# calmiLovesAI/ComputerVision.pytorch

Hardware: AMD Instinct MI355X
Metric: images/sec 640x640 YOLOv8-n train step (higher is better)
Workload: dtype f16; 1 GPU; YOLOv8-n train step (fwd + v8 loss + bwd + Adam), batch 32/GPU, 640x640, nc=80, random init; global_batch=32, parallelism=dp1, launch=eager, exchange=none (1 rank), gpu_max_hw_queues=4

## Files before the change

__graft_entry__.py:

```python
import os
import subprocess
import sys

ROOT = os.path.dirname(os.path.abspath(__file__))
CSRC = os.path.join(ROOT, "computervision.pytorch_amd", "csrc")
LIBDIR = os.path.join(ROOT, "computervision.pytorch_amd", "lib")
LIB = os.path.join(LIBDIR, "libcvx_engine.so")
SOURCES = ["conv_igemm.hip", "conv_igemm_dma.hip", "conv_halo.hip", "conv_tile.hip", "conv_tile_k1.hip", "conv_tile_k2.hip", "conv_gemm.hip", "conv_stem7.hip", "conv_pw.hip", "conv_wgrad.hip", "conv_wgrad_gemm.hip", "conv_wgrad_halo.hip", "conv_wgrad_stream.hip", "conv_wgrad_k3.hip", "bn_act.hip", "stem.hip", "unit_ops.hip", "misc_ops.hip", "loss_v8.hip", "loss_seg.hip", "loss_seg_opts.hip", "loss_centernet.hip", "loss_multibox.hip", "loss_yolov7.hip", "preprocess.hip", "augment.hip", "seg_pipeline.hip", "det_eval.hip", "coco_eval.hip", "nms.hip", "centernet_decode.hip", "render.hip", "tiles.hip", "seg_tiles.hip", "seg_tta.hip", "det_tta.hip", "track.hip", "optim.hip", "comm.hip", "engine.hip"]


def _stale(out, deps):
    if not os.path.exists(out):
        return True
    t = os.path.getmtime(out)
    return any(os.path.getmtime(d) > t for d in deps)


def build(force: bool = False) -> None:
    os.makedirs(LIBDIR, exist_ok=True)
    objdir = os.path.join(ROOT, "build", "obj")
    os.makedirs(objdir, exist_ok=True)
    headers = [os.path.join(CSRC, f) for f in os.listdir(CSRC) if f.endswith(".h")] + [os.path.join(ROOT, "include", "cvx_engine.h")]
    hipcc = os.environ.get("HIPCC", "/opt/rocm/bin/hipcc")
    objs, procs = [], []
    for src in SOURCES:
        s = os.path.join(CSRC, src)
        o = os.path.join(objdir, src.replace(".hip", ".o"))
        objs.append(o)
        if force or _stale(o, [s] + headers):
            cmd = [hipcc, "--offload-arch=gfx950", "-O3", "-std=c++17", "-fPIC", "-c", s, "-o", o]
            procs.append((src, subprocess.Popen(cmd, stdout=subprocess.PIPE, stderr=subprocess.STDOUT, text=True)))
    for src, p in procs:
        out, _ = p.communicate()
        if p.returncode != 0:
            raise RuntimeError(f"hipcc failed on {src}:\n{out}")
    if force or procs or _stale(LIB, objs):
        cmd = [hipcc, "--offload-arch=gfx950", "-shared", "-fPIC", "-o", LIB] + objs
        r = subprocess.run(cmd, stdout=subprocess.PIPE, stderr=subprocess.STDOUT, text=True)
        if r.returncode != 0:
            raise RuntimeError("link failed:\n" + r.stdout)
    if ROOT not in sys.path:
# ... 46 lines not shown
```

computervision.pytorch_amd/_lib.py:

```python
from __future__ import annotations

import ctypes as C
import os

import numpy as np

_HERE = os.path.dirname(os.path.abspath(__file__))
LIB_PATH = os.environ.get("CVX_LIB") or os.path.join(_HERE, "lib", "libcvx_engine.so")
ABI_VERSION = 4
SEG_OPTS_KEY_OFFSET = 4096


class CvxError(RuntimeError):
    pass


class BufDesc(C.Structure):
    _fields_ = [("h", C.c_int32), ("w", C.c_int32), ("c", C.c_int32), ("kind", C.c_int32)]


class View(C.Structure):
    _fields_ = [("buf", C.c_int32), ("coff", C.c_int32), ("c", C.c_int32), ("pix_off", C.c_int32)]


# ... 20 lines not shown

_P, _I32, _I64, _F, _U64 = C.c_void_p, C.c_int32, C.c_int64, C.c_float, C.c_uint64

EXPERIMENTAL_PROTOTYPES = {
    "cvx_chain_pair_unit": (_I32, [_P, _I32, _I32, _I32, _I32, _P, _P, _P, _P, _P, _P, _I32, _P, _I32, _I32, _I32, C.POINTER(_F), _P]),
    "cvx_chain_conv_unit": (_I32, [_P, _I32, _I32, _I32, _I32, _P, _I32, _I32, _I32, _I32, _P, _P, _I32, _P, _I32, _I32, _I32, C.POINTER(_F), _P]),
    "cvx_chain_detect_unit": (_I32, [_P, _I32, _I32, _I32, _I32, _I32, _I32, _I32, _P, _P, _P, _P, _P, _P, _P, _P, _P, _P, _P, _I32, _I32, _I32,
                                     _I32, _I32, C.POINTER(_F), _P]),
    "cvx_wgrad_time_unit": (_I32, [_P, _P, _I32, _I32, _I32, _I32, _I32, _I32, _I32, _I32, _I32, _I32, _P, _I64, C.POINTER(_F), C.POINTER(_I32), _P]),
}

PROTOTYPES = {
    "cvx_last_error": (C.c_char_p, []),
    "cvx_abi_version": (_I32, []),
    "cvx_engine_create": (_I32, [C.POINTER(_P), C.POINTER(BufDesc), _I32, C.POINTER(OpDesc), _I32, _I32, _I32, _I32, _P]),
    "cvx_engine_destroy": (_I32, [_P]),
    "cvx_engine_bind": (_I32, [_P, _P, _P, _I64, _P, _I64]),
    "cvx_engine_set_bn": (_I32, [_P, _F, _F]),
    "cvx_engine_forward": (_I32, [_P, _P, _I32, _I32, _P]),
    "cvx_engine_backward": (_I32, [_P, _P, _F]),
    "cvx_engine_backward_begin": (_I32, [_P, _P, _F]),
    "cvx_engine_backward_range": (_I32, [_P, _I32, _I32]),
    "cvx_engine_grads_ready": (_I32, [_P, _I32, _I32, _P]),
    "cvx_engine_backward_end": (_I32, [_P]),
    "cvx_engine_workspace_bytes": (_I64, [_P]),
    "cvx_engine_plan_generation": (_I64, [_P]),
    "cvx_engine_debug_copy": (_I32, [_P, _I32, _I32, _P, _I64]),
    "cvx_engine_profile": (_I32, [_P, _I32]),
    "cvx_engine_profile_read": (_I32, [_P, _I32, C.POINTER(C.c_double), C.POINTER(C.c_double), C.POINTER(C.c_double),
                                       C.POINTER(_I64)]),
    "cvx_debug_clock_buffer": (_I32, [_P]),
    "cvx_debug_conv_tile_plan": (_I32, [_I32, _I32, _I32, _I32, _I32, _P]),
    "cvx_debug_conv_dma_plan": (_I32, [_I64, _I32, _I32, _I32, _P]),
    "cvx_engine_profile_dump": (_I32, [_P, C.c_char_p]),
    "cvx_pred_level_to_nchw": (_I32, [_P, _I32, _I32, _I32, _I32, _I32, _I32, _P, _P]),
    "cvx_nchw_grad_to_dpred": (_I32, [_P, _I32, _I32, _I32, _I32, _I32, _I32, _F, _P, _P]),
    "cvx_loss_v8_workspace_bytes": (_I64, [_I32, _I32, _I32, _I32]),
    "cvx_loss_v8": (_I32, [_P, _I32, _I32, _I32, _P, _I32, _I32, C.POINTER(_I32), C.POINTER(_F), _I32, _F, _F, _F, _F, _P, _P, _P,
                           _I64, _P]),
    "cvx_loss_v8_strided": (_I32, [_P, _I32, _I32, _I32, _I32, _P, _I32, _I32, C.POINTER(_I32), C.POINTER(_F), _I32, _F, _F, _F, _F, _P, _P, _P,
                                   _I64, _P]),
    "cvx_loss_v8_assignment": (_I32, [_P, _I32, _I32, _I32, _P, _P, _P]),
    "cvx_pack_targets": (_I32, [_P, _P, _P, _I32, _P, _P]),
    "cvx_decode_strided": (_I32, [_P, _I32, _I32, _I32, _I32, C.POINTER(_I32), C.POINTER(_F), _I32, _P, _P]),
    "cvx_adam_step": (_I32, [_P, _P, _P, _P, _I64, _F, _F, _F, _F, _I32, _P, _I32, _P]),
    "cvx_check_finite": (_I32, [_P, _I64, _P, _P]),
    "cvx_adam_step_dev": (_I32, [_P, _P, _P, _P, _I64, _F, _F, _F, _P, _P, _I32, _F, _P]),
    "cvx_ema_update": (_I32, [_P, _P, _I64, _F, _F, _P]),
    "cvx_adam_ema_step_dev": (_I32, [_P, _P, _P, _P, _I64, _F, _F, _F, _P, _P, _I32, _F, _P, _F, _F, _P]),
    "cvx_optim_step": (_I32, [_I32, _P, _P, _P, _P, _I64, _P, _P, _I32, _P, _F, _F, _F, _P, _I32, _F, _P, _P, _F, _F, _P]),
    "cvx_grad_norm_workspace": (_I64, [_I64]),
    "cvx_grad_norm": (_I32, [_P, _I64, _P, _P, _I32, _F, _F, _P, _P, _P, _I64, _P]),
    "cvx_engine_set_stream": (_I32, [_P, _P]),
    "cvx_engine_exchange_stream": (_P, [_P]),
    "cvx_decode": (_I32, [_P, _I32, _I32, _I32, C.POINTER(_I32), C.POINTER(_F), _I32, _P, _P]),
    "cvx_yolo7_decode": (_I32, [_P, _I32, _I32, _I32, _P, _P, _I32, _I32, _I32, _P, _P, _P]),
    "cvx_ssd_decode": (_I32, [_P, _P, _P, _I32, _I32, _I32, _F, _F, _P, _P, _P]),
    "cvx_ssd_decode_max": (_I32, [_P, _P, _P, _I32, _I32, _I32, _F, _F, _P, _P, _P, _P]),
    "cvx_pred_cols_to_nchw": (_I32, [_P, _I32, _I32, _I32, _I32, _I32, _I32, _I32, _P, _I64, _I64, _P]),
    "cvx_nms_workspace_bytes": (_I64, [_I32, _I32]),
    "cvx_nms": (_I32, [_P, _I32, _I32, _I32, _F, _F, _I32, _P, _P, _P, _P, _I64, _P]),
    "cvx_nms_variant": (_I32, [_P, _I32, _I32, _I32, _F, _F, _I32, _I32, _P, _P, _P, _P, _I64, _P]),
    "cvx_centernet_decode_workspace_bytes": (_I64, [_I32, _I32, _I32, _I32]),
    "cvx_centernet_decode": (_I32, [_P, _I32, _I32, _I32, _I32, _I32, _I32, _I32, _I32, _F, _F, _I32, _P, _P, _P, _P, _P, _P, _P, _I64, _P]),
    "cvx_conv2d_nhwc": (_I32, [_P, _I32, _I32, _I32, _I32, _P, _I32, _I32, _I32, _I32, _I32, _I32, _P, _P, _P, _P]),
    "cvx_conv2d_dgrad_nhwc": (_I32, [_P, _I32, _I32, _I32, _I32, _P, _I32, _I32, _I32, _I32, _I32, _P, _P]),
    "cvx_conv2d_wgrad_workspace_bytes": (_I64, [_I32, _I32, _I32, _I32, _I32, _I32]),
    "cvx_conv2d_wgrad_nhwc": (_I32, [_P, _P, _I32, _I32, _I32, _I32, _I32, _I32, _I32, _I32, _I32, _P, _P, _I64, _P]),
    "cvx_bn_silu_train_nhwc": (_I32, [_P, _I32, _I32, _I32, _P, _P, _F, _F, _P, _P, _P, _P, _P, _P, _P, _P]),
    "cvx_bn_silu_bwd_nhwc": (_I32, [_P, _P, _I32, _I32, _I32, _P, _P, _P, _F, _P, _P, _P, _P, _I32, _P]),
    "cvx_letterbox_geometry": (_I32, [_I32, _I32, _I32, _I32, _P, _P, _P, _P, _P]),
    "cvx_letterbox_u8_to_nchw": (_I32, [_P, _I32, _I32, _I32, _I32, _P, _I32, _I32, _P]),
    "cvx_letterbox_batch_u8_to_nchw": (_I32, [_P, _I32, _I32, _I32, _P, _I32, _I32, _P]),
    "cvx_det_to_image": (_I32, [_P, _P, _I32, _I32, _I32, _P, _P, _P, _P, _P]),
    "cvx_draw_detections": (_I32, [_P, _I32, _I32, _I32, _P, _P, _I32, _P, _I32, _I32, _I32, _P]),
    "cvx_seg_overlay": (_I32, [_P, _I32, _I32, _I32, _P, _I32, _I32, _I32, _I32, _I32, _I32, _P, _I32, _P]),
    "cvx_tiles_u8_to_nchw": (_I32, [_P, _I32, _I32, _P, _I32, _I32, _P]),
    "cvx_det_merge_workspace_bytes": (_I64, [_I32]),
    "cvx_det_merge_tiles": (_I32, [_P, _P, _I32, _I32, _P, _P, _I32, _I32, _F, _I32, _I32, _P, _P, _P, _P, _P, _I64, _P]),
    "cvx_track_state_bytes": (_I64, [_I32]),
    "cvx_track_update": (_I32, [_P, _P, _I32, _I32, _P, _I32, _P, _P, _P, _P, _P]),
    "cvx_draw_tracks": (_I32, [_P, _I32, _I32, _I32, _P, _P, _I32, _P, _P, _I32, _I32, _I32, _P]),
    "cvx_seg_stitch": (_I32, [_P, _I32, _I32, _I32, _I32, _I32, _I32, _I32, _P, _P, _I32, _P, _I32, _I32, _I32, _P, _P, _P, _P, _I32, _I32, _I32, _P]),
    "cvx_seg_tta_inputs": (_I32, [_P, _I32, _I32, _I32, _I32, _I32, _I32, _I32, _P, _P]),
    "cvx_seg_fuse": (_I32, [_P, _I32, _I32, _I32, _I32, _I32, _I32, _I32, _P, _P, _P, _P, _P]),
    "cvx_det_tta_inputs": (_I32, [_P, _I32, _I32, _I32, _P, _I32, _F, _P, _P]),
    "cvx_det_fuse_views": (_I32, [_P, _P, _I32, _P, _P, _I32, _I32, _F, _I32, _I32, _I32, _I32, _P, _P, _P, _P, _P, _P, _I64, _P]),
    "cvx_aug_images": (_I32, [_P, _P, _P, _I32, _P, _I32, _I32, _P]),
    "cvx_aug_boxes": (_I32, [_P, _P, _I32, _P, _I32, _I32, _I32, _P, _P, _P]),
    "cvx_aug_images_plain": (_I32, [_P, _P, _I32, _P, _I32, _I32, _P]),
    "cvx_aug_boxes_padded": (_I32, [_P, _P, _P, _I32, _P, _I32, _I32, _I32, _I32, _P, _P, _P, _P]),
    "cvx_aug_warp_mix": (_I32, [_P, _P, _I32, _P, _I32, _I32, _P]),
    "cvx_aug_boxes_warp": (_I32, [_P, _P, _I32, _P, _I32, _I32, _I32, _F, _F, _F, _I32, _P, _I32, _P, _P, _P]),
    "cvx_engine_set_seed": (_I32, [_P, _U64]),
    "cvx_engine_keep_shadows": (_I32, [_P]),
    "cvx_engine_set_fusion": (_I32, [_P, _I32]),
    "cvx_engine_fused_groups": (_I32, [_P]),
    "cvx_centernet_loss_workspace_bytes": (_I64, [_I32, _I32]),
# ... 104 lines not shown
```

computervision.pytorch_amd/csrc/conv_igemm.h:

```cpp
#pragma once
#include "cvx_common.h"
#include "bn_act.h"
#include "conv_plan.h"

enum {
  CVX_EPI_RAW_STATS = 0,
  CVX_EPI_AFFINE_SILU = 1,
  CVX_EPI_BIAS_F32 = 2,
  CVX_EPI_PLAIN = 3,
};

#define CVX_MAX_TAPS 64

struct ConvParams {
  const half_t* in;
  long long in_bstride;
  int in_ld;
  int IH, IW;
  int Cin;
  const half_t* wt;
  int wt_ld;
  int Cout;
  int B, OH2, OW2;
  int IS;
// ... 21 lines not shown
  int dbg;
  unsigned long long* clk;
  int halo_taps_ok;
  int nphase;
  struct Phase {
    const ConvTap* taps;
    int ntaps, OH2, OW2, oph, opw;
  } phase[4];
  int pointwise;
  unsigned long long halo_pos, halo_wt;
  const half_t* wt_packed;
  int wt_packed_bn, wt_packed_kc;
  int std7x7;
  int std3x3;
  int gemm_variant;
  const half_t* tile_packed;
  int tile_packed_bn;
  int no_tile;
  int ps_cin;
  int raw16;
};

__device__ __forceinline__ void cvx_store_raw4(const ConvParams& p, long long off, const f4& v) {
  if (p.raw16) *reinterpret_cast<h4*>(p.out16 + off) = h4{(half_t)v[0], (half_t)v[1], (half_t)v[2], (half_t)v[3]};
  else *reinterpret_cast<f4*>(p.out32 + off) = v;
}

extern unsigned long long* g_cvx_clk;
extern int g_cvx_grid_div;
int cvx_conv_igemm_launch(const ConvParams& p, hipStream_t stream);
int cvx_conv_igemm_dma_launch(const ConvParams& p, hipStream_t stream);
bool cvx_conv_halo_supported(const ConvParams& p);
int cvx_conv_halo_launch(const ConvParams& p, hipStream_t stream);
bool cvx_conv_stem7_supported(const ConvParams& p);
int cvx_conv_stem7_launch(const ConvParams& p, hipStream_t stream);
struct GemmPackJob {
  const half_t* src;
  half_t* dst;
  const ConvTap* taps;
  int src_ld, rows, Cin, ntaps, BN, kc, nblocks, chunks;
  int blk0, nblk;
};
bool cvx_conv_gemm_plan(const ConvParams& p, GemmPackJob* job, size_t* bytes);
int cvx_conv_gemm_pack_jobs(const GemmPackJob* d_jobs, int njobs, int nblocks, hipStream_t stream);
bool cvx_conv_gemm_shape_ok(const ConvParams& p);
bool cvx_conv_gemm_supported(const ConvParams& p);
int cvx_conv_gemm_launch(const ConvParams& p, hipStream_t stream);
void cvx_conv_gemm_release();
struct TilePackPlan {
  int BN, NB, SPT;
  size_t bytes;
  double cost_us;
};
bool cvx_conv_tile_shape_ok(const ConvParams& p);
bool cvx_conv_tile_supported(const ConvParams& p);
bool cvx_conv_tile_plan(const ConvParams& p, TilePackPlan* out);
int cvx_conv_tile_fill_job(const ConvParams& p, const TilePackPlan& tp, half_t* dst, int blk0, void* job_out);
size_t cvx_conv_tile_job_bytes();
int cvx_conv_tile_pack_jobs(const void* d_jobs, int njobs, int nblocks, hipStream_t stream);
int cvx_conv_tile_launch(const ConvParams& p, hipStream_t stream);
void cvx_conv_tile_release();
bool cvx_conv_pw_supported(const ConvParams& p);
int cvx_conv_pw_launch(const ConvParams& p, hipStream_t stream);

struct WgradParams {
  const half_t* x;
// ... 32 lines not shown
```

computervision.pytorch_amd/csrc/conv_igemm.hip:

```cpp
#include "conv_igemm.h"

unsigned long long* g_cvx_clk = nullptr;
int g_cvx_grid_div = 1;

int cvx_conv_igemm_launch(const ConvParams& p_in, hipStream_t stream) {
  ConvParams p = p_in;
  p.clk = g_cvx_clk;
  CVX_CHECK(p.Cin % 8 == 0 && p.in_ld % 8 == 0 && p.wt_ld % 8 == 0, "conv: channel counts must be multiples of 8");
  CVX_CHECK(p.Cout % 4 == 0 && p.out_ld % 4 == 0, "conv: Cout/out_ld must be multiples of 4");
  CVX_CHECK(p.ntaps >= 1 && p.ntaps <= CVX_MAX_TAPS, "conv: bad tap count");
  CVX_CHECK(((uintptr_t)p.in % 16) == 0 && ((uintptr_t)p.wt % 16) == 0, "conv: operands must be 16-byte aligned");
  CVX_CHECK(p.zeros && ((uintptr_t)p.zeros % 16) == 0, "conv: needs a 16-byte aligned zero page (padding source of the LDS DMA)");
  CVX_CHECK((long long)p.B * p.OH2 * p.OW2 > 0, "conv: empty output");
  if (p.ps_cin > 0) {
    CVX_CHECK(p.epi == CVX_EPI_PLAIN && p.nphase <= 1 && p.OS == 2 && p.oph == 0 && p.opw == 0 && p.ps_cin % 8 == 0 && p.Cout == 4 * p.ps_cin &&
                  cvx_conv_gemm_shape_ok(p),
              "conv: pixel-shuffle data gradient needs the GEMM-shaped kernel (plain epilogue, 4 phases of ps_cin channels, output stride 2)");
    return cvx_conv_gemm_launch(p, stream);
  }
  if (p.nphase > 1) return cvx_conv_igemm_dma_launch(p, stream);
  if (cvx_conv_stem7_supported(p)) return cvx_conv_stem7_launch(p, stream);
  if (cvx_conv_tile_supported(p)) return cvx_conv_tile_launch(p, stream);
  if (cvx_conv_gemm_supported(p)) return cvx_conv_gemm_launch(p, stream);
  if (cvx_conv_pw_supported(p)) return cvx_conv_pw_launch(p, stream);
  if (cvx_conv_halo_supported(p)) return cvx_conv_halo_launch(p, stream);
  return cvx_conv_igemm_dma_launch(p, stream);
}
```

computervision.pytorch_amd/csrc/engine.hip:

```cpp
#include <algorithm>
#include <atomic>
#include <cstdlib>
#include <cstdio>
#include <cstring>
#include <vector>

#include "../../include/cvx_engine.h"
#ifdef CVX_WITH_CHAIN
#include "conv_chain.h"
#endif
#include "bn_act.h"
#include "conv_igemm.h"
#include <map>
#include <mutex>

#include "misc_ops.h"
#include "stem.h"

static unsigned cvx_event_flags() {
  static const bool sysfence = cvx_tune_set("CVX_EVENT_SYSFENCE");
  return hipEventDisableTiming | (sysfence ? 0u : hipEventDisableSystemFence);
}

static thread_local std::string g_last_error;
// ... 2272 lines not shown
  std::vector<void*> ptrs;
  DevTemps() = default;
  DevTemps(const DevTemps&) = delete;
  DevTemps& operator=(const DevTemps&) = delete;
  ~DevTemps() {
    for (void* p : ptrs) (void)hipFree(p);
  }
  template <typename T>
  int alloc(T** out, size_t bytes) {
    void* p = nullptr;
    CVX_HIP(hipMalloc(&p, bytes));
    ptrs.push_back(p);
    *out = (T*)p;
    return 0;
  }
  int taps(const std::vector<ConvTap>& host, const ConvTap** dev, const half_t** zeros = nullptr) {
    const size_t tb = ((host.size() * sizeof(ConvTap) + 255) / 256) * 256;
    char* p = nullptr;
    CVX_TRY(alloc(&p, tb + 256));
    CVX_HIP(hipMemset(p, 0, tb + 256));
    CVX_HIP(hipMemcpy(p, host.data(), host.size() * sizeof(ConvTap), hipMemcpyHostToDevice));
    *dev = reinterpret_cast<const ConvTap*>(p);
    if (zeros) *zeros = reinterpret_cast<const half_t*>(p + tb);
    return 0;
  }
};
ViewDesc dense_view(const void* p, long long pixels, int c) { return ViewDesc{(half_t*)p, pixels * c, c}; }
long long unit_wgrad_splits(long long M) { return std::min<long long>(std::max<long long>(1, M / 256), 64); }
}

extern "C" int cvx_conv2d_nhwc(const void* x_f16, int32_t batch, int32_t ih, int32_t iw, int32_t cin, const void* w_f16, int32_t cout,
                               int32_t k, int32_t stride, int32_t pad, int32_t dil, int32_t mode, const float* scale_or_bias,
                               const float* shift, void* out, void* hip_stream) {
  CVX_CHECK(x_f16 && w_f16 && out && k * k <= CVX_MAX_TAPS && stride >= 1 && dil >= 1, "bad arguments");
  hipStream_t st = (hipStream_t)hip_stream;
  const bool force_gemm = (mode & 0x100) != 0;
  const int gemm_variant = (mode >> 9) & 15;
  const bool force_tile = (mode & 0x2000) != 0;
  const bool no_tile = (mode & 0x4000) != 0;
  const bool force_dma = (mode & 0x8000) != 0;
  mode &= 0xff;
  const int oh = cvx_conv_out_size(ih, k, stride, pad, dil), ow = cvx_conv_out_size(iw, k, stride, pad, dil);
  const std::vector<ConvTap> taps = cvx_conv_fwd_taps(k, pad, dil);
  DevTemps tmp;
  const ConvTap* dt = nullptr;
  const half_t* zeros = nullptr;
  CVX_TRY(tmp.taps(taps, &dt, &zeros));
  ConvParams cp;
  fill_conv_fwd(ConvGeom{batch, ih, iw, cin, oh, ow, cout, stride, k * k}, dense_view(x_f16, (long long)ih * iw, cin), (const half_t*)w_f16, dt,
                cvx_tap_traits(taps), zeros, &cp);
  cp.out_ld = cout;
  cp.out_bstride = (long long)oh * ow * cout;
  if (mode == 0) {
    cp.epi = CVX_EPI_PLAIN;
    cp.out16 = (half_t*)out;
  } else if (mode == 1) {
    cp.epi = CVX_EPI_AFFINE_SILU;
    cp.scale = scale_or_bias;
    cp.shift = shift;
    cp.out16 = (half_t*)out;
  } else if (mode == 2) {
    cp.epi = CVX_EPI_BIAS_F32;
    cp.bias = scale_or_bias;
    cp.out32 = (float*)out;
  } else {
    CVX_CHECK(shift, "mode 3 needs the statistics slab (cvx_stat_replicas(cout) * cout * 4 64-bit words, zeroed) in `shift`");
    cp.epi = CVX_EPI_RAW_STATS;
    cp.out32 = (float*)out;
    cp.stats = (long long*)shift;
    cp.stats_replicas = cvx_stat_replicas(cout);
  }
  int rc;
  cp.gemm_variant = gemm_variant;
  if (force_gemm) {
    CVX_CHECK(cvx_conv_gemm_shape_ok(cp), "shape outside the GEMM-shaped kernel (cin % 8, cout % 4)");
    rc = cvx_conv_gemm_launch(cp, st);
  } else if (force_tile) {
    CVX_CHECK(cvx_conv_tile_shape_ok(cp), "shape outside the row-band kernel (3x3 stride 1, cin % 8, cin >= 32)");
    cp.clk = g_cvx_clk;
    rc = cvx_conv_tile_launch(cp, st);
  } else if (force_dma) {
    CVX_CHECK(cin % 8 == 0 && cout % 4 == 0 && oh > 0 && ow > 0 && batch > 0, "shape outside the ring kernel (cin % 8, cout % 4, a non-empty output)");
    CVX_CHECK(((uintptr_t)x_f16 % 16) == 0 && ((uintptr_t)w_f16 % 16) == 0, "conv: operands must be 16-byte aligned");
    cp.clk = g_cvx_clk;
    rc = cvx_conv_igemm_dma_launch(cp, st);
  } else {
    cp.no_tile = no_tile ? 1 : 0;
    rc = cvx_conv_igemm_launch(cp, st);
  }
  (void)hipStreamSynchronize(st);
  return rc;
}

extern "C" int cvx_conv2d_dgrad_nhwc(const void* dy_f16, int32_t batch, int32_t ih, int32_t iw, int32_t cin, const void* wt_f16, int32_t cout,
                                     int32_t k, int32_t stride, int32_t pad, int32_t dil, void* dx_f16, void* hip_stream) {
  CVX_CHECK(dy_f16 && wt_f16 && dx_f16 && k * k <= CVX_MAX_TAPS && stride >= 1 && stride <= 4, "bad arguments");
  hipStream_t st = (hipStream_t)hip_stream;
  const int oh = cvx_conv_out_size(ih, k, stride, pad, dil), ow = cvx_conv_out_size(iw, k, stride, pad, dil);
  const ConvGeom g{batch, ih, iw, cin, oh, ow, cout, stride, k * k};
  const ViewDesc dy = dense_view(dy_f16, (long long)oh * ow, cout), dx = dense_view(dx_f16, (long long)ih * iw, cin);
  const std::vector<DgradPhase> phases = cvx_conv_dgrad_phases(k, stride, pad, dil, ih, iw);
// ... 132 lines not shown
```

include/cvx_engine.h:

```cpp
#ifndef CVX_ENGINE_H
#define CVX_ENGINE_H
#include <stdint.h>
#ifdef __cplusplus
extern "C" {
#endif

#define CVX_ABI_VERSION 4

const char* cvx_last_error(void);
int cvx_abi_version(void);

enum { CVX_BUF_ACT_F16 = 0, CVX_BUF_PRED_F32 = 1 };
typedef struct {
  int32_t h, w, c;
  int32_t kind;
} cvx_buf_desc;

typedef struct {
  int32_t buf;
  int32_t coff;
  int32_t c;
  int32_t pix_off;
} cvx_view;

// ... 39 lines not shown
int cvx_engine_destroy(cvx_engine* e);

int cvx_engine_bind(cvx_engine* e, float* params, float* grads, int64_t n_params, float* stats, int64_t n_stats);

int cvx_engine_set_stream(cvx_engine* e, void* hip_stream);
void* cvx_engine_exchange_stream(cvx_engine* e);

int cvx_engine_set_bn(cvx_engine* e, float eps, float momentum);
int cvx_engine_keep_shadows(cvx_engine* e);
int cvx_engine_set_fusion(cvx_engine* e, int32_t enable);
int32_t cvx_engine_fused_groups(const cvx_engine* e);

int cvx_engine_set_seed(cvx_engine* e, uint64_t seed);

int cvx_engine_forward(cvx_engine* e, const float* images, int32_t batch, int32_t training, float* pred);

int cvx_engine_backward(cvx_engine* e, const void* dpred_f16, float loss_scale);

int cvx_engine_debug_copy(cvx_engine* e, int32_t buf, int32_t which, void* dst, int64_t bytes);

int cvx_engine_backward_begin(cvx_engine* e, const void* dpred_f16, float loss_scale);
int cvx_engine_backward_range(cvx_engine* e, int32_t op_hi, int32_t op_lo);
int cvx_engine_grads_ready(cvx_engine* e, int32_t op_hi, int32_t op_lo, void* hip_stream);
int cvx_engine_backward_end(cvx_engine* e);

int cvx_engine_profile(cvx_engine* e, int32_t enable);
int cvx_engine_profile_read(cvx_engine* e, int32_t n_classes, double* ms, double* flops, double* bytes, int64_t* launches);
int cvx_engine_profile_dump(cvx_engine* e, const char* path);

int cvx_debug_clock_buffer(void* buf);

int cvx_debug_conv_tile_plan(int32_t batch, int32_t h, int32_t w, int32_t cin, int32_t cout, int32_t* out8);
int cvx_debug_conv_dma_plan(int64_t pixels, int32_t cin, int32_t cout, int32_t ntaps, int32_t* out4);

int64_t cvx_engine_workspace_bytes(const cvx_engine* e);
int64_t cvx_engine_plan_generation(const cvx_engine* e);

int cvx_pred_level_to_nchw(const float* pred, int32_t batch, int32_t anchors, int32_t no, int32_t a_off, int32_t h, int32_t w,
                           float* out_nchw, void* hip_stream);
int cvx_nchw_grad_to_dpred(const float* grad_nchw, int32_t batch, int32_t anchors, int32_t no, int32_t a_off, int32_t h, int32_t w,
                           float scale, void* dpred_f16, void* hip_stream);

int64_t cvx_loss_v8_workspace_bytes(int32_t batch, int32_t anchors, int32_t nc, int32_t max_targets_per_image);
int cvx_loss_v8(const float* pred, int32_t batch, int32_t anchors, int32_t nc, const float* targets, int32_t n_targets,
                int32_t max_targets_per_image, const int32_t* level_hw, const float* strides, int32_t n_levels, float gain_box,
                float gain_cls, float gain_dfl, float loss_scale, float* loss_items, void* dpred_f16, void* workspace,
                int64_t workspace_bytes, void* hip_stream);
int cvx_loss_v8_strided(const float* pred, int32_t pred_ld, int32_t batch, int32_t anchors, int32_t nc, const float* targets,
                        int32_t n_targets, int32_t max_targets_per_image, const int32_t* level_hw, const float* strides, int32_t n_levels,
                        float gain_box, float gain_cls, float gain_dfl, float loss_scale, float* loss_items, void* dpred_f16,
                        void* workspace, int64_t workspace_bytes, void* hip_stream);

int cvx_loss_v8_assignment(const void* workspace, int32_t batch, int32_t anchors, int32_t max_targets_per_image, int32_t* gt_index,
                           float* norm_score, void* hip_stream);
int cvx_pack_targets(const float* batch_idx, const float* cls, const float* bboxes, int32_t n, float* rows, void* hip_stream);

int cvx_letterbox_geometry(int32_t h, int32_t w, int32_t H, int32_t W, int32_t* new_h, int32_t* new_w, int32_t* top, int32_t* left, double* scale);
int cvx_letterbox_u8_to_nchw(const uint8_t* image_hwc, int32_t h, int32_t w, int32_t letterbox, int32_t swap_rb, float* out_chw, int32_t H,
                             int32_t W, void* hip_stream);
typedef struct cvx_letterbox_job {
  const uint8_t* src;
  int32_t h, w, out, reserved;
} cvx_letterbox_job;
int cvx_letterbox_batch_u8_to_nchw(const cvx_letterbox_job* jobs, int32_t n_jobs, int32_t letterbox, int32_t swap_rb, float* out_nchw, int32_t H,
                                   int32_t W, void* hip_stream);

// ... 21 lines not shown

int cvx_decode(const float* pred, int32_t batch, int32_t anchors, int32_t nc, const int32_t* level_hw, const float* strides,
               int32_t n_levels, float* y, void* hip_stream);
int cvx_decode_strided(const float* pred, int32_t pred_ld, int32_t batch, int32_t anchors, int32_t nc, const int32_t* level_hw,
                       const float* strides, int32_t n_levels, float* y, void* hip_stream);
int cvx_ssd_decode(const float* loc, const float* conf, const float* priors, int32_t batch, int32_t anchors, int32_t num_classes_plus_bg,
                   float variance_xy, float variance_wh, float* boxes, float* prob, void* hip_stream);
int cvx_ssd_decode_max(const float* loc, const float* conf, const float* priors, int32_t B, int32_t A, int32_t num_classes_plus_bg,
                       float variance_xy, float variance_wh, float* boxes, float* prob, float* class_max, void* hip_stream);
int cvx_pred_cols_to_nchw(const float* rows, int32_t ld, int32_t col0, int32_t c, int32_t batch, int32_t anchors, int32_t a_off, int32_t hw,
                          float* out, int64_t out_bstride, int64_t out_off, void* hip_stream);
int cvx_yolo7_decode(const float* pred, int32_t pred_ld, int32_t batch, int32_t nc, const int32_t* level_hw, const float* anchors_wh,
                     int32_t n_levels, int32_t input_h, int32_t input_w, float* dec, float* y, void* hip_stream);
enum { CVX_NMS_TV0141_CUDA = 0,
       CVX_NMS_TV0141_CPU = 1,
       CVX_NMS_OFFSET = 2,
       CVX_NMS_VANILLA = 3 };
#define CVX_NMS_BOXES_XYXY 0x100
int64_t cvx_nms_workspace_bytes(int32_t batch, int32_t anchors);
int cvx_nms(const float* y, int32_t batch, int32_t anchors, int32_t nc, float conf_thres, float iou_thres, int32_t max_det,
            float* out_rows, int32_t* out_index, int32_t* counts, void* workspace, int64_t workspace_bytes, void* hip_stream);
int cvx_nms_variant(const float* y, int32_t batch, int32_t anchors, int32_t nc, float conf_thres, float iou_thres, int32_t max_det,
                    int32_t variant, float* out_rows, int32_t* out_index, int32_t* counts, void* workspace, int64_t workspace_bytes,
                    void* hip_stream);

int64_t cvx_centernet_decode_workspace_bytes(int32_t batch, int32_t h, int32_t w, int32_t nc);
int cvx_centernet_decode(const float* pred, int32_t pred_ld, int32_t batch, int32_t h, int32_t w, int32_t nc, int32_t reg_col, int32_t wh_col,
                         int32_t k, float conf, float nms_thr, int32_t use_nms, float* boxes, float* scores, int32_t* classes,
                         int32_t* topk_index, int32_t* keep, int32_t* counts, void* workspace, int64_t workspace_bytes, void* hip_stream);

int cvx_conv2d_nhwc(const void* x_f16, int32_t batch, int32_t ih, int32_t iw, int32_t cin, const void* w_f16, int32_t cout, int32_t k,
                    int32_t stride, int32_t pad, int32_t dil, int32_t mode, const float* scale_or_bias, const float* shift, void* out,
                    void* hip_stream);
int cvx_conv2d_dgrad_nhwc(const void* dy_f16, int32_t batch, int32_t ih, int32_t iw, int32_t cin, const void* wt_f16, int32_t cout,
                          int32_t k, int32_t stride, int32_t pad, int32_t dil, void* dx_f16, void* hip_stream);
int64_t cvx_conv2d_wgrad_workspace_bytes(int32_t batch, int32_t oh, int32_t ow, int32_t cin, int32_t cout, int32_t k);
int cvx_conv2d_wgrad_nhwc(const void* x_f16, const void* dy_f16, int32_t batch, int32_t ih, int32_t iw, int32_t cin, int32_t cout,
                          int32_t k, int32_t stride, int32_t pad, int32_t dil, float* dw, void* workspace, int64_t workspace_bytes,
                          void* hip_stream);


int cvx_bn_silu_train_nhwc(const float* y_f32, int32_t batch, int32_t hw, int32_t c, const float* gamma, const float* beta, float eps,
                           float momentum, float* running_mean, float* running_var, const void* res_f16, void* out_f16, void* xhat_f16,
                           float* mean, float* invstd, void* hip_stream);
int cvx_bn_silu_bwd_nhwc(const void* xhat_f16, const void* gout_f16, int32_t batch, int32_t hw, int32_t c, const float* gamma,
                         const float* beta, const float* invstd, float inv_scale, float* dgamma, float* dbeta, void* dy_f16, void* gres_f16,
                         int32_t res_accumulate, void* hip_stream);
int cvx_bn_act_train_nhwc(const float* y_f32, int32_t batch, int32_t hw, int32_t c, const float* gamma, const float* beta, float eps,
                          float momentum, float* running_mean, float* running_var, const void* res_f16, int32_t act, int32_t res_pre,
                          void* out_f16, void* xhat_f16, float* mean, float* invstd, void* hip_stream);
int cvx_bn_act_bwd_nhwc(const void* xhat_f16, const void* gout_f16, const void* out_f16, int32_t batch, int32_t hw, int32_t c,
                        const float* gamma, const float* beta, const float* invstd, int32_t act, int32_t res_pre, float inv_scale,
                        float* dgamma, float* dbeta, void* dy_f16, void* gres_f16, int32_t res_accumulate, void* hip_stream);
int cvx_maxpool5_nhwc(const void* x_f16, int32_t batch, int32_t h, int32_t w, int32_t c, void* out_f16, uint8_t* argmax, void* hip_stream);
int cvx_maxpool5_bwd_nhwc(const void* gout_f16, const uint8_t* argmax, int32_t batch, int32_t h, int32_t w, int32_t c, void* gin_f16,
                          int32_t accumulate, void* hip_stream);
int cvx_maxpool_nhwc(const void* x_f16, int32_t batch, int32_t h, int32_t w, int32_t c, int32_t kernel, int32_t stride, int32_t ceil_mode,
                     void* out_f16, void* hip_stream);
int cvx_avgpool_global_nhwc(const void* x_f16, int32_t batch, int32_t hw, int32_t c, void* out_f16, void* hip_stream);
int cvx_resize_bilinear_nhwc(const void* x_f16, int32_t batch, int32_t ih, int32_t iw, int32_t c, int32_t oh, int32_t ow, void* out_f16,
                             void* hip_stream);
int cvx_l2norm_nhwc(const void* x_f16, const float* weight, int32_t batch, int32_t hw, int32_t c, void* out_f16, void* hip_stream);
int cvx_resize_bilinear_rows_to_nchw(const float* rows_f32, int32_t ld, int32_t batch, int32_t c, int32_t ih, int32_t iw, int32_t oh, int32_t ow,
                                     float* out_nchw, void* hip_stream);
int64_t cvx_seg_loss_workspace_bytes(int32_t batch, int32_t nc, int32_t oh, int32_t ow);
int cvx_seg_loss(const float* rows_f32, int32_t ld, int32_t batch, int32_t nc, int32_t ih, int32_t iw, int32_t oh, int32_t ow,
// ... 221 lines not shown
```

Baseline: 5643 images/sec.

## Add dedicated stride-2 3x3 conv kernel with LDS patch staging

```diff
diff --git a/__graft_entry__.py b/__graft_entry__.py
--- a/__graft_entry__.py
+++ b/__graft_entry__.py
@@ -6,7 +6,7 @@
 CSRC = os.path.join(ROOT, "computervision.pytorch_amd", "csrc")
 LIBDIR = os.path.join(ROOT, "computervision.pytorch_amd", "lib")
 LIB = os.path.join(LIBDIR, "libcvx_engine.so")
-SOURCES = ["conv_igemm.hip", "conv_igemm_dma.hip", "conv_halo.hip", "conv_tile.hip", "conv_tile_k1.hip", "conv_tile_k2.hip", "conv_gemm.hip", "conv_stem7.hip", "conv_pw.hip", "conv_wgrad.hip", "conv_wgrad_gemm.hip", "conv_wgrad_halo.hip", "conv_wgrad_stream.hip", "conv_wgrad_k3.hip", "bn_act.hip", "stem.hip", "unit_ops.hip", "misc_ops.hip", "loss_v8.hip", "loss_seg.hip", "loss_seg_opts.hip", "loss_centernet.hip", "loss_multibox.hip", "loss_yolov7.hip", "preprocess.hip", "augment.hip", "seg_pipeline.hip", "det_eval.hip", "coco_eval.hip", "nms.hip", "centernet_decode.hip", "render.hip", "tiles.hip", "seg_tiles.hip", "seg_tta.hip", "det_tta.hip", "track.hip", "optim.hip", "comm.hip", "engine.hip"]
+SOURCES = ["conv_igemm.hip", "conv_igemm_dma.hip", "conv_halo.hip", "conv_s2.hip", "conv_tile.hip", "conv_tile_k1.hip", "conv_tile_k2.hip", "conv_gemm.hip", "conv_stem7.hip", "conv_pw.hip", "conv_wgrad.hip", "conv_wgrad_gemm.hip", "conv_wgrad_halo.hip", "conv_wgrad_stream.hip", "conv_wgrad_k3.hip", "bn_act.hip", "stem.hip", "unit_ops.hip", "misc_ops.hip", "loss_v8.hip", "loss_seg.hip", "loss_seg_opts.hip", "loss_centernet.hip", "loss_multibox.hip", "loss_yolov7.hip", "preprocess.hip", "augment.hip", "seg_pipeline.hip", "det_eval.hip", "coco_eval.hip", "nms.hip", "centernet_decode.hip", "render.hip", "tiles.hip", "seg_tiles.hip", "seg_tta.hip", "det_tta.hip", "track.hip", "optim.hip", "comm.hip", "engine.hip"]
 
 
 def _stale(out, deps):
diff --git a/computervision.pytorch_amd/_lib.py b/computervision.pytorch_amd/_lib.py
--- a/computervision.pytorch_amd/_lib.py
+++ b/computervision.pytorch_amd/_lib.py
@@ -76,6 +76,7 @@
     "cvx_debug_clock_buffer": (_I32, [_P]),
     "cvx_debug_conv_tile_plan": (_I32, [_I32, _I32, _I32, _I32, _I32, _P]),
     "cvx_debug_conv_dma_plan": (_I32, [_I64, _I32, _I32, _I32, _P]),
+    "cvx_debug_conv_s2_plan": (_I32, [_I32, _I32, _I32, _I32, _I32, _I32, _I32, _I32, _I32, _P]),
     "cvx_engine_profile_dump": (_I32, [_P, C.c_char_p]),
     "cvx_pred_level_to_nchw": (_I32, [_P, _I32, _I32, _I32, _I32, _I32, _I32, _P, _P]),
     "cvx_nchw_grad_to_dpred": (_I32, [_P, _I32, _I32, _I32, _I32, _I32, _I32, _F, _P, _P]),
@@ -108,6 +109,7 @@
     "cvx_centernet_decode_workspace_bytes": (_I64, [_I32, _I32, _I32, _I32]),
     "cvx_centernet_decode": (_I32, [_P, _I32, _I32, _I32, _I32, _I32, _I32, _I32, _I32, _F, _F, _I32, _P, _P, _P, _P, _P, _P, _P, _I64, _P]),
     "cvx_conv2d_nhwc": (_I32, [_P, _I32, _I32, _I32, _I32, _P, _I32, _I32, _I32, _I32, _I32, _I32, _P, _P, _P, _P]),
+    "cvx_conv2d_nhwc_view": (_I32, [_P, _I32, _I32, _I32, _I32, _I32, _P, _I32, _I32, _I32, _I32, _I32, _I32, _I32, _P, _P, _P, _P]),
     "cvx_conv2d_dgrad_nhwc": (_I32, [_P, _I32, _I32, _I32, _I32, _P, _I32, _I32, _I32, _I32, _I32, _P, _P]),
     "cvx_conv2d_wgrad_workspace_bytes": (_I64, [_I32, _I32, _I32, _I32, _I32, _I32]),
     "cvx_conv2d_wgrad_nhwc": (_I32, [_P, _P, _I32, _I32, _I32, _I32, _I32, _I32, _I32, _I32, _I32, _P, _P, _I64, _P]),
diff --git a/computervision.pytorch_amd/csrc/conv_igemm.h b/computervision.pytorch_amd/csrc/conv_igemm.h
--- a/computervision.pytorch_amd/csrc/conv_igemm.h
+++ b/computervision.pytorch_amd/csrc/conv_igemm.h
@@ -77,6 +77,8 @@
 int cvx_conv_igemm_dma_launch(const ConvParams& p, hipStream_t stream);
 bool cvx_conv_halo_supported(const ConvParams& p);
 int cvx_conv_halo_launch(const ConvParams& p, hipStream_t stream);
+bool cvx_conv_s2_supported(const ConvParams& p);
+int cvx_conv_s2_launch(const ConvParams& p, hipStream_t stream);
 bool cvx_conv_stem7_supported(const ConvParams& p);
 int cvx_conv_stem7_launch(const ConvParams& p, hipStream_t stream);
 struct GemmPackJob {
diff --git a/computervision.pytorch_amd/csrc/conv_igemm.hip b/computervision.pytorch_amd/csrc/conv_igemm.hip
--- a/computervision.pytorch_amd/csrc/conv_igemm.hip
+++ b/computervision.pytorch_amd/csrc/conv_igemm.hip
@@ -24,5 +24,6 @@
   if (cvx_conv_gemm_supported(p)) return cvx_conv_gemm_launch(p, stream);
   if (cvx_conv_pw_supported(p)) return cvx_conv_pw_launch(p, stream);
   if (cvx_conv_halo_supported(p)) return cvx_conv_halo_launch(p, stream);
+  if (cvx_conv_s2_supported(p)) return cvx_conv_s2_launch(p, stream);
   return cvx_conv_igemm_dma_launch(p, stream);
 }
diff --git a/computervision.pytorch_amd/csrc/conv_s2.hip b/computervision.pytorch_amd/csrc/conv_s2.hip
--- /dev/null
+++ b/computervision.pytorch_amd/csrc/conv_s2.hip
@@ -0,0 +1,324 @@
+#include <cstdlib>
+#include <type_traits>
+
+#include "conv_tile_common.h"
+
+namespace {
+using namespace cvx_tile;
+
+constexpr int PW = 33;
+constexpr int LDS_CU = 160 * 1024;
+
+template <int I, int N, typename F>
+__device__ __forceinline__ void static_for(F&& f) {
+  if constexpr (I < N) {
+    f(std::integral_constant<int, I>{});
+    static_for<I + 1, N>(f);
+  }
+}
+
+template <int WM, int WN, int MT, int NTW, int CIN_, int HV_>
+struct S2Geom {
+  static constexpr int HV = HV_;
+  static constexpr int CIN = CIN_;
+  static constexpr int P = CIN >> 3;
+  static constexpr int TH = WM * MT;
+  static constexpr int BN = 16 * NTW * WN;
+  static constexpr int NPIECE = BN / 16;
+  static constexpr int PB = (NPIECE + 4 * HV_ - 1) / (4 * HV_);
+  static constexpr int STEP_HALVES = BN * BK;
+  static constexpr int NSTEPS = (9 * CIN + BK - 1) / BK;
+  static constexpr int UNITS = (2 * TH + 1) * PW * P;
+  static constexpr int PATCH_PIECES = (UNITS + 63) / 64;
+  static constexpr int STAT_BYTES = HV_ * WM * BN * 2 * 4;
+  static constexpr int WGS_CU = HV_ == 2 ? 1 : (BN <= 32 ? 3 : 2);
+  static constexpr int LDS_BYTES = (2 * HV_ * PATCH_PIECES + 1) * 1024 + NSTEPS * STEP_HALVES * 2 + STAT_BYTES;
+};
+
+template <int P>
+__device__ __forceinline__ int slot_swz(int q) {
+  constexpr int SH = P == 2 ? 3 : P == 4 ? 2 : 1;
+  return (q >> SH) & (P - 1);
+}
+
+template <int WM, int WN, int MT, int NTW, int CIN, int HV>
+__global__ __launch_bounds__(256 * HV, (S2Geom<WM, WN, MT, NTW, CIN, HV>::WGS_CU)) void conv_s2_kernel(const ConvParams p, int tiles_x, int tiles_y, int total_tiles) {
+  using G = S2Geom<WM, WN, MT, NTW, CIN, HV>;
+  constexpr int TH = G::TH, BN = G::BN, PB = G::PB, Cin = G::CIN, P = G::P, NSTEPS = G::NSTEPS;
+  constexpr int PER_WAVE = (G::PATCH_PIECES + 3) / 4;
+  extern __shared__ __attribute__((aligned(16))) unsigned char smem[];
+  half_t* patch0 = reinterpret_cast<half_t*>(smem);
+  half_t* patch_dump = patch0 + 2 * HV * G::PATCH_PIECES * 512;
+  half_t* wts = patch_dump + 512;
+  float* sStat = reinterpret_cast<float*>(wts + NSTEPS * G::STEP_HALVES);
+
+  const int tid = threadIdx.x;
+  const int wave8 = __builtin_amdgcn_readfirstlane(tid >> 6), lane = tid & 63;
+  const int half = wave8 >> 2, wave = wave8 & 3;
+  const int wm = wave / WN, wn = wave % WN;
+  const int fr = lane & 15, fq = lane >> 4;
+  const int nblk = blockIdx.y;
+  const int H = p.IH, W = p.IW, OH = p.OH2, OW = p.OW2;
+  clk_mark(p, 0);
+
+  int prel[PER_WAVE], prc[PER_WAVE];
+#pragma unroll
+  for (int k = 0; k < PER_WAVE; ++k) {
+    const int u = (k * 4 + wave) * 64 + lane;
+    const int hp = u / P, phys = u - hp * P;
+    const int pr = hp / PW, q = hp - pr * PW;
+    const int pc = q < 17 ? 2 * q : 2 * (q - 17) + 1;
+    prel[k] = (pr * W + pc) * p.in_ld + ((phys ^ slot_swz<P>(q)) << 3);
+    prc[k] = u < G::UNITS ? (pr << 8) | pc : (0x4000 << 8);
+  }
+  auto issue_patch = [&](int tile, int buf) {
+    const int tx = tile % tiles_x;
+    const int t2 = tile / tiles_x;
+    const int ty = t2 % tiles_y;
+    const int b = t2 / tiles_y;
+    const int iy0 = 2 * ty * TH - 1, ix0 = 2 * tx * 16 - 1;
+    const long long origin = (long long)b * p.in_bstride + ((long long)iy0 * W + ix0) * p.in_ld;
+    half_t* pbuf = patch0 + (half * 2 + buf) * (G::PATCH_PIECES * 512);
+#pragma unroll
+    for (int k = 0; k < PER_WAVE; ++k) {
+      const int piece = k * 4 + wave;
+      const int iy = iy0 + (prc[k] >> 8), ix = ix0 + (prc[k] & 255);
+      const bool in_image = (unsigned)iy < (unsigned)H && (unsigned)ix < (unsigned)W;
+      const half_t* g = in_image ? p.in + (origin + prel[k]) : p.zeros;
+      half_t* dst = piece < G::PATCH_PIECES ? pbuf + piece * 512 : patch_dump;
+      __builtin_amdgcn_global_load_lds((gbl_void_ptr)g, (lds_void_ptr)dst, 16, 0, 0);
+    }
+  };
+
+  const int tstride = gridDim.x * HV;
+  int tile = blockIdx.x * HV + half;
+  bool valid = tile < total_tiles;
+  auto dump_patch = [&]() {
+#pragma unroll
+    for (int k = 0; k < PER_WAVE; ++k) __builtin_amdgcn_global_load_lds((gbl_void_ptr)p.zeros, (lds_void_ptr)patch_dump, 16, 0, 0);
+  };
+  if (valid) issue_patch(tile, 0);
+  else dump_patch();
+
+  const unsigned long long pos_pack = p.halo_pos, wt_pack = p.halo_wt;
+
+  {
+    const int r16 = lane >> 2;
+    const int kg = (lane & 3) ^ ((r16 >> 1) & 3);
+    const half_t* wrow[PB];
+    half_t* wdst[PB];
+#pragma unroll
+    for (int q = 0; q < PB; ++q) {
+      const int piece = q * (4 * HV) + wave8;
+      const int n = nblk * BN + piece * 16 + r16;
+      wrow[q] = (piece < G::NPIECE && n < p.Cout) ? p.wt + (long long)n * p.wt_ld : nullptr;
+      wdst[q] = piece < G::NPIECE ? wts + piece * 512 : nullptr;
+    }
+    for (int s = 0; s < NSTEPS; ++s) {
+      const int k = s * BK + kg * 8;
+      const int tapb = k / Cin, cb = k - tapb * Cin;
+      const bool kvalid = tapb < 9;
+      const int wtap = (int)(wt_pack >> (4 * (kvalid ? tapb : 0))) & 15;
+#pragma unroll
+      for (int q = 0; q < PB; ++q) {
+        const half_t* g = (kvalid && wrow[q]) ? wrow[q] + wtap * Cin + cb : p.zeros;
+        half_t* dst = wdst[q] ? wdst[q] + s * G::STEP_HALVES : patch_dump;
+        __builtin_amdgcn_global_load_lds((gbl_void_ptr)g, (lds_void_ptr)dst, 16, 0, 0);
+      }
+    }
+  }
+  clk_mark(p, 1);
+
+  const int xrow = 2 * wm * PW;
+  const half_t* wbase = wts + lds_row_off(wn * NTW * 16 + fr, fq);
+  f4 st1[NTW], st2[NTW];
+#pragma unroll
+  for (int j = 0; j < NTW; ++j) st1[j] = st2[j] = f4{0.f, 0.f, 0.f, 0.f};
+
+  constexpr int NG = NSTEPS >= 12 ? 3 : (NSTEPS >= 4 ? 2 : 1);
+  bool first = true;
+  int buf = 0;
+  for (int tile0 = blockIdx.x * HV; tile0 < total_tiles; tile0 += tstride, tile += tstride, buf ^= 1) {
+    valid = tile < total_tiles;
+    const int next = tile + tstride;
+    const bool has_next = tile0 + tstride < total_tiles;
+    const bool next_valid = next < total_tiles;
+    f4 acc[MT][NTW];
+#pragma unroll
+    for (int i = 0; i < MT; ++i)
+#pragma unroll
+      for (int j = 0; j < NTW; ++j) acc[i][j] = f4{0.f, 0.f, 0.f, 0.f};
+    const half_t* patch = patch0 + (half * 2 + buf) * (G::PATCH_PIECES * 512);
+    const int tx = tile % tiles_x;
+    const int t2 = tile / tiles_x;
+    const int ty = t2 % tiles_y;
+    const int b = t2 / tiles_y;
+    long long out_off[MT], res_off[MT];
+    bool pvalid[MT];
+#pragma unroll
+    for (int i = 0; i < MT; ++i) {
+      const int oy = ty * TH + i * WM + wm, ox = tx * 16 + fr;
+      pvalid[i] = oy < OH && ox < OW;
+      const long long pix = pvalid[i] ? (long long)oy * p.OWr + ox : 0;
+      out_off[i] = (long long)b * p.out_bstride + pix * p.out_ld;
+      res_off[i] = (long long)b * p.res_bstride + pix * p.res_ld;
+    }
+
+    static_for<0, NG>([&](auto gi) {
+      constexpr int g = decltype(gi)::value;
+      constexpr int beg = (NSTEPS * g) / NG, end = (NSTEPS * (g + 1)) / NG;
+      if (g == 0 || first) {
+        constexpr int pend = (NSTEPS - end) * PB;
+        if (first) {
+          if (g > 0 && has_next) wait_vmcnt<(pend + PER_WAVE > 63 ? 63 : pend + PER_WAVE)>();
+          else wait_vmcnt<(pend > 63 ? 63 : pend)>();
+        }
+        workgroup_barrier();
+        if (g == 0) {
+          if (first) clk_mark(p, 2);
+          if (has_next) {
+            if (next_valid) issue_patch(next, buf ^ 1);
+            else dump_patch();
+          }
+        }
+      }
+      constexpr int PD = 2;
+      h8 xa[PD + 1][MT], wb[PD + 1][NTW];
+      auto load_step = [&](auto si) {
+        constexpr int s = decltype(si)::value;
+        constexpr int slot = (s - beg) % (PD + 1);
+        auto tap_slot = [&](int tp) {
+          const int code = (int)(pos_pack >> (4 * tp)) & 15;
+          const int dh = code >> 2, dw = code & 3;
+          return dh * 64 + (dw == 1 ? 17 : (dw >> 1));
+        };
+        int chunk, rs;
+        if constexpr (Cin >= BK) {
+          chunk = (((BK * s) % Cin) >> 3) + fq;
+          rs = tap_slot((BK * s) / Cin);
+        } else {
+          chunk = fq & 1;
+          rs = (fq & 2) ? tap_slot(2 * s + 1 > 8 ? 0 : 2 * s + 1) : tap_slot(2 * s);
+        }
+        const int q = fr + (rs & 63);
+        const half_t* xp = patch + (((xrow + (rs >> 6) * PW + q) * P + (chunk ^ slot_swz<P>(q))) << 3);
+#pragma unroll
+        for (int i = 0; i < MT; ++i) xa[slot][i] = *reinterpret_cast<const h8*>(xp + i * 2 * WM * PW * P * 8);
+#pragma unroll
+        for (int j = 0; j < NTW; ++j) wb[slot][j] = *reinterpret_cast<const h8*>(wbase + s * G::STEP_HALVES + j * 16 * BK);
+      };
+      static_for<beg, (beg + PD < end ? beg + PD : end)>(load_step);
+      static_for<beg, end>([&](auto si) {
+        constexpr int s = decltype(si)::value;
+        constexpr int slot = (s - beg) % (PD + 1);
+        if constexpr (s + PD < end) load_step(std::integral_constant<int, s + PD>{});
+        __builtin_amdgcn_sched_barrier(0);
+#pragma unroll
+        for (int j = 0; j < NTW; ++j)
+#pragma unroll
+          for (int i = 0; i < MT; ++i) acc[i][j] = __builtin_amdgcn_mfma_f32_16x16x32_f16(wb[slot][j], xa[slot][i], acc[i][j], 0, 0, 0);
+        __builtin_amdgcn_sched_barrier(0);
+      });
+    });
+    if (first) clk_mark(p, 3);
+
+    if (has_next) wait_vmcnt<0>();
+    if (valid) epilogue_tile<WM, WN, MT, NTW>(p, acc, out_off, res_off, pvalid, wn, fq, nblk, st1, st2);
+    first = false;
+  }
+  if (p.epi == CVX_EPI_RAW_STATS) stats_flush<HV * WM, WN, NTW>(p, st1, st2, half * WM + wm, wn, fr, fq, nblk, sStat, tid);
+  clk_mark(p, 4);
+}
+
+
+int s2_lds_bytes(int th, int wm, int bn, int cin, int hv) {
+  const int pieces = ((2 * th + 1) * PW * (cin / 8) + 63) / 64;
+  const int nsteps = (9 * cin + BK - 1) / BK;
+  return (2 * hv * pieces + 1) * 1024 + nsteps * bn * BK * 2 + hv * wm * bn * 2 * 4;
+}
+
+struct S2Plan {
+  int th, wm, bn, hv, lds, gx, gy, per_cu;
+};
+bool s2_plan(int B, int ih, int iw, int cin, int cout, S2Plan* pl) {
+  if (!(cin == 16 || cin == 32 || cin == 64) || cout < 4 || cout % 4 != 0 || B < 1 || ih < 1 || iw < 1) return false;
+  const int oh = (ih - 1) / 2 + 1, ow = (iw - 1) / 2 + 1;
+  const int tiles = (cout + 15) / 16;
+  if (cin == 64) {
+    pl->th = 2, pl->wm = 2, pl->hv = 2;
+    pl->bn = tiles <= 2 ? 32 : 64;
+  } else {
+    pl->th = cin == 16 ? 8 : 4, pl->wm = 4, pl->hv = 1;
+    pl->bn = tiles <= 1 ? 16 : (tiles <= 2 ? 32 : 64);
+  }
+  pl->gy = (cout + pl->bn - 1) / pl->bn;
+  pl->lds = s2_lds_bytes(pl->th, pl->wm, pl->bn, cin, pl->hv);
+  int per_cu = LDS_CU / pl->lds;
+  if (per_cu * 4 * pl->hv < 8) return false;
+  const int reg_cu = pl->hv == 2 ? 1 : (pl->bn <= 32 ? 3 : 2);
+  if (per_cu > reg_cu) per_cu = reg_cu;
+  pl->per_cu = per_cu;
+  const long long total = (long long)((ow + 15) / 16) * ((oh + pl->th - 1) / pl->th) * B;
+  if (total > 0x7fffffff / 64 || ih >= 0x4000 || iw >= 0x4000) return false;
+  int gx = (256 * per_cu) / pl->gy / (g_cvx_grid_div > 0 ? g_cvx_grid_div : 1);
+  if (gx < 1) gx = 1;
+  if ((long long)gx * pl->hv > total) gx = (int)((total + pl->hv - 1) / pl->hv);
+  pl->gx = gx;
+  return true;
+}
+
+template <int WM, int WN, int MT, int NTW, int CIN, int HV>
+int launch_s2(const ConvParams& p, hipStream_t stream, const S2Plan& pl) {
+  using G = S2Geom<WM, WN, MT, NTW, CIN, HV>;
+  CVX_CHECK(G::LDS_BYTES == pl.lds && G::TH == pl.th && G::BN == pl.bn && pl.lds <= LDS_CU && pl.per_cu <= G::WGS_CU, "conv_s2: plan and kernel geometry disagree or exceed the LDS (launcher bug)");
+  const int tiles_x = (p.OW2 + 15) / 16, tiles_y = (p.OH2 + G::TH - 1) / G::TH;
+  const int total = tiles_x * tiles_y * p.B;
+  static unsigned long long optin_mask = 0;
+  CVX_TRY(cvx_lds_optin((const void*)conv_s2_kernel<WM, WN, MT, NTW, CIN, HV>, G::LDS_BYTES, &optin_mask));
+  hipLaunchKernelGGL((conv_s2_kernel<WM, WN, MT, NTW, CIN, HV>), dim3(pl.gx, pl.gy), dim3(256 * HV), G::LDS_BYTES, stream, p, tiles_x, tiles_y, total);
+  return 0;
+}
+
+bool s2_geometry_ok(int ih, int iw, int oh, int ow) { return oh == (ih - 1) / 2 + 1 && ow == (iw - 1) / 2 + 1; }
+
+}
+
+bool cvx_conv_s2_supported(const ConvParams& p) {
+  static const bool off = cvx_tune_set("CVX_NO_S2");
+  if (off || !p.zeros) return false;
+  if (p.IS != 2 || p.OS != 1 || p.oph != 0 || p.opw != 0 || p.nphase > 1 || p.ps_cin != 0) return false;
+  if (p.ntaps != 9 || !p.halo_taps_ok || !p.std3x3) return false;
+  if (!s2_geometry_ok(p.IH, p.IW, p.OH2, p.OW2) || p.OWr != p.OW2) return false;
+  if (18LL * p.IW * p.in_ld > 0x7fffffff) return false;
+  S2Plan pl;
+  return s2_plan(p.B, p.IH, p.IW, p.Cin, p.Cout, &pl);
+}
+
+int cvx_conv_s2_launch(const ConvParams& p, hipStream_t stream) {
+  S2Plan pl;
+  CVX_CHECK(s2_plan(p.B, p.IH, p.IW, p.Cin, p.Cout, &pl), "conv_s2: shape outside the kernel (dispatcher bug)");
+  const int key = p.Cin * 1000 + pl.bn;
+  switch (key) {
+    case 16016: CVX_TRY((launch_s2<4, 1, 2, 1, 16, 1>(p, stream, pl))); break;
+    case 16032: CVX_TRY((launch_s2<4, 1, 2, 2, 16, 1>(p, stream, pl))); break;
+    case 16064: CVX_TRY((launch_s2<4, 1, 2, 4, 16, 1>(p, stream, pl))); break;
+    case 32016: CVX_TRY((launch_s2<4, 1, 1, 1, 32, 1>(p, stream, pl))); break;
+    case 32032: CVX_TRY((launch_s2<4, 1, 1, 2, 32, 1>(p, stream, pl))); break;
+    case 32064: CVX_TRY((launch_s2<4, 1, 1, 4, 32, 1>(p, stream, pl))); break;
+    case 64032: CVX_TRY((launch_s2<2, 2, 1, 1, 64, 2>(p, stream, pl))); break;
+    case 64064: CVX_TRY((launch_s2<2, 2, 1, 2, 64, 2>(p, stream, pl))); break;
+    default: CVX_CHECK(false, "conv_s2: no compiled configuration for the plan (launcher bug)");
+  }
+  CVX_HIP(hipGetLastError());
+  return 0;
+}
+
+extern "C" int cvx_debug_conv_s2_plan(int32_t batch, int32_t ih, int32_t iw, int32_t cin, int32_t cout, int32_t k, int32_t stride, int32_t pad,
+                                      int32_t dil, int32_t* out5) {
+  CVX_CHECK(out5 && batch >= 1 && ih >= 1 && iw >= 1 && cin >= 1 && cout >= 1, "bad arguments");
+  for (int i = 0; i < 5; ++i) out5[i] = 0;
+  S2Plan pl;
+  if (k != 3 || stride != 2 || pad != 1 || dil != 1 || !s2_plan(batch, ih, iw, cin, cout, &pl)) return 0;
+  out5[0] = pl.th, out5[1] = pl.bn, out5[2] = pl.hv, out5[3] = pl.lds, out5[4] = pl.gx * pl.gy;
+  return 0;
+}
diff --git a/computervision.pytorch_amd/csrc/engine.hip b/computervision.pytorch_amd/csrc/engine.hip
--- a/computervision.pytorch_amd/csrc/engine.hip
+++ b/computervision.pytorch_amd/csrc/engine.hip
@@ -2328,7 +2328,15 @@
 extern "C" int cvx_conv2d_nhwc(const void* x_f16, int32_t batch, int32_t ih, int32_t iw, int32_t cin, const void* w_f16, int32_t cout,
                                int32_t k, int32_t stride, int32_t pad, int32_t dil, int32_t mode, const float* scale_or_bias,
                                const float* shift, void* out, void* hip_stream) {
+  CVX_CHECK((mode & 0xff) <= 3, "bad mode");
+  return cvx_conv2d_nhwc_view(x_f16, batch, ih, iw, cin, cin, w_f16, cout, cout, k, stride, pad, dil, mode, scale_or_bias, shift, out, hip_stream);
+}
+
+extern "C" int cvx_conv2d_nhwc_view(const void* x_f16, int32_t batch, int32_t ih, int32_t iw, int32_t cin, int32_t in_ld, const void* w_f16,
+                                    int32_t cout, int32_t out_ld, int32_t k, int32_t stride, int32_t pad, int32_t dil, int32_t mode,
+                                    const float* scale_or_bias, const float* shift, void* out, void* hip_stream) {
   CVX_CHECK(x_f16 && w_f16 && out && k * k <= CVX_MAX_TAPS && stride >= 1 && dil >= 1, "bad arguments");
+  CVX_CHECK(in_ld >= cin && out_ld >= cout && in_ld % 8 == 0 && out_ld % 4 == 0 && (mode & 0xff) <= 4, "bad slice strides or mode");
   hipStream_t st = (hipStream_t)hip_stream;
   const bool force_gemm = (mode & 0x100) != 0;
   const int gemm_variant = (mode >> 9) & 15;
@@ -2343,10 +2351,10 @@
   const half_t* zeros = nullptr;
   CVX_TRY(tmp.taps(taps, &dt, &zeros));
   ConvParams cp;
-  fill_conv_fwd(ConvGeom{batch, ih, iw, cin, oh, ow, cout, stride, k * k}, dense_view(x_f16, (long long)ih * iw, cin), (const half_t*)w_f16, dt,
+  fill_conv_fwd(ConvGeom{batch, ih, iw, cin, oh, ow, cout, stride, k * k}, ViewDesc{(half_t*)x_f16, (long long)ih * iw * in_ld, in_ld}, (const half_t*)w_f16, dt,
                 cvx_tap_traits(taps), zeros, &cp);
-  cp.out_ld = cout;
-  cp.out_bstride = (long long)oh * ow * cout;
+  cp.out_ld = out_ld;
+  cp.out_bstride = (long long)oh * ow * out_ld;
   if (mode == 0) {
     cp.epi = CVX_EPI_PLAIN;
     cp.out16 = (half_t*)out;
@@ -2363,6 +2371,8 @@
     CVX_CHECK(shift, "mode 3 needs the statistics slab (cvx_stat_replicas(cout) * cout * 4 64-bit words, zeroed) in `shift`");
     cp.epi = CVX_EPI_RAW_STATS;
     cp.out32 = (float*)out;
+    cp.out16 = (half_t*)out;
+    cp.raw16 = mode == 4 ? 1 : 0;
     cp.stats = (long long*)shift;
     cp.stats_replicas = cvx_stat_replicas(cout);
   }
diff --git a/include/cvx_engine.h b/include/cvx_engine.h
--- a/include/cvx_engine.h
+++ b/include/cvx_engine.h
@@ -95,6 +95,8 @@
 
 int cvx_debug_conv_tile_plan(int32_t batch, int32_t h, int32_t w, int32_t cin, int32_t cout, int32_t* out8);
 int cvx_debug_conv_dma_plan(int64_t pixels, int32_t cin, int32_t cout, int32_t ntaps, int32_t* out4);
+int cvx_debug_conv_s2_plan(int32_t batch, int32_t ih, int32_t iw, int32_t cin, int32_t cout, int32_t k, int32_t stride, int32_t pad,
+                           int32_t dil, int32_t* out5);
 
 int64_t cvx_engine_workspace_bytes(const cvx_engine* e);
 int64_t cvx_engine_plan_generation(const cvx_engine* e);
@@ -182,6 +184,9 @@
 int cvx_conv2d_nhwc(const void* x_f16, int32_t batch, int32_t ih, int32_t iw, int32_t cin, const void* w_f16, int32_t cout, int32_t k,
                     int32_t stride, int32_t pad, int32_t dil, int32_t mode, const float* scale_or_bias, const float* shift, void* out,
                     void* hip_stream);
+int cvx_conv2d_nhwc_view(const void* x_f16, int32_t batch, int32_t ih, int32_t iw, int32_t cin, int32_t in_ld, const void* w_f16, int32_t cout,
+                         int32_t out_ld, int32_t k, int32_t stride, int32_t pad, int32_t dil, int32_t mode, const float* scale_or_bias,
+                         const float* shift, void* out, void* hip_stream);
 int cvx_conv2d_dgrad_nhwc(const void* dy_f16, int32_t batch, int32_t ih, int32_t iw, int32_t cin, const void* wt_f16, int32_t cout,
                           int32_t k, int32_t stride, int32_t pad, int32_t dil, void* dx_f16, void* hip_stream);
 int64_t cvx_conv2d_wgrad_workspace_bytes(int32_t batch, int32_t oh, int32_t ow, int32_t cin, int32_t cout, int32_t k);
```

After: 5695 images/sec, median of 6. Within noise of the previous version (+0.9%).
